# yahoo/bftkv

Hardware: NVIDIA H100
Metric: rsa2048_signature_verifies_per_sec (higher is better)
Workload: dtype u32 limbs / u64 products (integer)

## Files before the change

### bftkv_b200/csrc/rsa_square_r32.cuh

```cuda
#pragma once
#include <cstdint>
#include <cuda_runtime.h>

namespace bftq {
namespace r32 {

__device__ __forceinline__ void mad_pair_first(uint32_t& lo, uint32_t& hi, const uint32_t x, const uint32_t m) {
  asm volatile("mad.lo.cc.u32 %0, %2, %3, %0; madc.hi.cc.u32 %1, %2, %3, %1;" : "+r"(lo), "+r"(hi) : "r"(x), "r"(m));
}
__device__ __forceinline__ void mad_pair_next(uint32_t& lo, uint32_t& hi, const uint32_t x, const uint32_t m) {
  asm volatile("madc.lo.cc.u32 %0, %2, %3, %0; madc.hi.cc.u32 %1, %2, %3, %1;" : "+r"(lo), "+r"(hi) : "r"(x), "r"(m));
}
template <int N>
__device__ __forceinline__ void chain_n(uint32_t* p, uint32_t& c0, uint32_t& c1, const uint32_t* x, const uint32_t m, const uint32_t t) {
  if (N == 0) {
    asm volatile("add.cc.u32 %0, %0, %2; addc.u32 %1, %1, 0;" : "+r"(c0), "+r"(c1) : "r"(t));
    return;
  }
  mad_pair_first(p[0], p[1], x[0], m);
#pragma unroll
  for (int i = 1; i < N; i++) mad_pair_next(p[2 * i], p[2 * i + 1], x[2 * i], m);
  asm volatile("addc.cc.u32 %0, %0, %2; addc.u32 %1, %1, 0;" : "+r"(c0), "+r"(c1) : "r"(t));
}
template <int N>
__device__ __forceinline__ void chain_n1(uint32_t* p, uint32_t& c, const uint32_t* x, const uint32_t m) {
  mad_pair_first(p[0], p[1], x[0], m);
#pragma unroll
  for (int i = 1; i < N; i++) mad_pair_next(p[2 * i], p[2 * i + 1], x[2 * i], m);
  asm volatile("addc.u32 %0, %0, 0;" : "+r"(c));
}

template <int JJ>
__device__ __forceinline__ void sqr_iter(Acc<16>& A, uint32_t& cy1, const uint32_t (&a2)[17], const uint32_t (&n)[16],
                                         const uint32_t n0inv, const int r, const int gbase, const int owner) {
  constexpr int W = 16;
  const uint32_t lt1 = r < owner ? ~1u : 0u, nm = r < owner ? ~0u : ~1u, eqm = r == owner ? ~0u : 0u;
  const uint32_t aj0 = __funnelshift_r(a2[JJ], a2[JJ + 1], 1);
  const uint32_t aj1 = __funnelshift_r(a2[JJ + 1], a2[JJ + 2], 1);
  const uint32_t b0 = __shfl_sync(kFull, aj0, gbase + owner);
  const uint32_t b1 = __shfl_sync(kFull, aj1, gbase + owner);
  uint32_t m0[18], m1[18];
#pragma unroll
  for (int k = 0; k < 17; k++) { m0[k] = a2[k]; m1[k] = a2[k]; }
  m0[17] = 0u; m1[17] = 0u;
  m0[JJ] = (a2[JJ] & lt1) | (aj0 & eqm);
  m0[JJ + 1] = a2[JJ + 1] & nm;
  m1[JJ + 1] = (a2[JJ + 1] & lt1) | (aj1 & eqm);
  uint32_t top1 = a2[16];
  if (JJ + 2 < W) m1[JJ + 2] = a2[JJ + 2] & nm;
  else top1 = a2[16] & (lt1 >> 1);
  const uint32_t t0 = (0u - a2[16]) & b0;
  const uint32_t t1 = (0u - top1) & b1;
  chain_n<(W - JJ) / 2>(A.E + JJ, A.E[W], A.E[W + 1], m0 + JJ, b0, t0);
  uint32_t q0 = A.E[0] * n0inv;
  q0 = __shfl_sync(kFull, q0, gbase);
  chain_n<(W - JJ) / 2>(A.O + JJ, A.O[W], A.O[W + 1], m0 + JJ + 1, b0, 0u);
  chain_n<(W - JJ - 2) / 2>(A.O + JJ + 2, A.O[W], A.O[W + 1], m1 + JJ + 2, b1, t1);
  chain_n1<(W - JJ) / 2>(A.E + JJ + 2, A.O[W + 1], m1 + JJ + 1, b1);
  mac_off0_even_nocin(A, n, q0);
  mac_off0_odd(A, n, q0);
  uint32_t q1 = (A.E[1] + A.O[0] + cy1) * n0inv;
  q1 = __shfl_sync(kFull, q1, gbase);
  Chain<W>::run_cin(A.O, A.O[W], A.O[W + 1], n, q1, cy1);
  chain_n1<W / 2>(A.E + 2, A.O[W + 1], n + 1, q1);
  const uint32_t p0 = A.E[0];
  uint32_t p1, e0;
  asm("add.cc.u32 %0, %3, %4; addc.cc.u32 %1, %5, %6; addc.u32 %2, 0, 0;"
      : "=r"(p1), "=r"(e0), "=r"(cy1) : "r"(A.E[1]), "r"(A.O[0]), "r"(A.E[2]), "r"(A.O[1]));
  uint32_t r0 = __shfl_down_sync(kFull, p0, 1, T);
  uint32_t r1 = __shfl_down_sync(kFull, p1, 1, T);
  if (r == T - 1) { r0 = 0u; r1 = 0u; }
#pragma unroll
  for (int k = 1; k < W; k++) A.E[k] = A.E[k + 2];
  A.E[0] = e0; A.E[W] = 0u; A.E[W + 1] = 0u;
#pragma unroll
  for (int k = 0; k < W; k++) A.O[k] = A.O[k + 2];
  A.O[W] = 0u; A.O[W + 1] = 0u;
  asm volatile("add.cc.u32 %0, %0, %3; addc.cc.u32 %1, %1, %4; addc.u32 %2, %2, 0;"
               : "+r"(A.E[W - 2]), "+r"(A.E[W - 1]), "+r"(A.O[W - 1]) : "r"(r0), "r"(r1));
}

__device__ __forceinline__ void mont_sqr(uint32_t (&out)[16], const uint32_t (&a)[16], const uint32_t (&n)[16], const uint32_t n0inv,
                                         const int r, const int gbase) {
  constexpr int W = 16;
  uint32_t a2[17];
  a2[0] = a[0] << 1;
#pragma unroll
  for (int k = 1; k < W; k++) a2[k] = __funnelshift_l(a[k - 1], a[k], 1);
  a2[16] = a[W - 1] >> 31;
  Acc<W> A;
#pragma unroll
  for (int k = 0; k < W + 4; k++) A.E[k] = 0u;
#pragma unroll
  for (int k = 0; k < W + 2; k++) A.O[k] = 0u;
  uint32_t cy1 = 0u;
#pragma unroll 2
  for (int owner = 0; owner < T; owner++) {
    sqr_iter<0>(A, cy1, a2, n, n0inv, r, gbase, owner);
    sqr_iter<2>(A, cy1, a2, n, n0inv, r, gbase, owner);
    sqr_iter<4>(A, cy1, a2, n, n0inv, r, gbase, owner);
    sqr_iter<6>(A, cy1, a2, n, n0inv, r, gbase, owner);
    sqr_iter<8>(A, cy1, a2, n, n0inv, r, gbase, owner);
    sqr_iter<10>(A, cy1, a2, n, n0inv, r, gbase, owner);
    sqr_iter<12>(A, cy1, a2, n, n0inv, r, gbase, owner);
    sqr_iter<14>(A, cy1, a2, n, n0inv, r, gbase, owner);
  }
  asm volatile("add.cc.u32 %0, %0, %1;" : "+r"(A.O[0]) : "r"(cy1));
#pragma unroll
  for (int k = 1; k < W; k++) asm volatile("addc.cc.u32 %0, %0, 0;" : "+r"(A.O[k]));
  mont_finish(out, A, 0u, 0u, n, r, gbase);
}

}
}
```

### bftkv_b200/csrc/rsa_verify_r32.cuh

```cuda
#pragma once
#include <cstdint>
#include <cuda_runtime.h>
#include "rsa_verify.cuh"

namespace bftq {
namespace r32 {

constexpr int T = 4;

#define BFTQ_CHAIN8_BODY(first)                                                              \
  first " %0, %18, %26, %0;  madc.hi.cc.u32 %1, %18, %26, %1;"                                \
  "madc.lo.cc.u32 %2, %19, %26, %2;  madc.hi.cc.u32 %3, %19, %26, %3;"                        \
  "madc.lo.cc.u32 %4, %20, %26, %4;  madc.hi.cc.u32 %5, %20, %26, %5;"                        \
  "madc.lo.cc.u32 %6, %21, %26, %6;  madc.hi.cc.u32 %7, %21, %26, %7;"                        \
  "madc.lo.cc.u32 %8, %22, %26, %8;  madc.hi.cc.u32 %9, %22, %26, %9;"                        \
  "madc.lo.cc.u32 %10, %23, %26, %10; madc.hi.cc.u32 %11, %23, %26, %11;"                     \
  "madc.lo.cc.u32 %12, %24, %26, %12; madc.hi.cc.u32 %13, %24, %26, %13;"                     \
  "madc.lo.cc.u32 %14, %25, %26, %14; madc.hi.cc.u32 %15, %25, %26, %15;"                     \
  "addc.cc.u32 %16, %16, 0; addc.u32 %17, %17, 0;"
#define BFTQ_CHAIN8_OPS(p, c0, c1, x)                                                                                     \
  : "+r"(p[0]), "+r"(p[1]), "+r"(p[2]), "+r"(p[3]), "+r"(p[4]), "+r"(p[5]), "+r"(p[6]), "+r"(p[7]), "+r"(p[8]), "+r"(p[9]), \
    "+r"(p[10]), "+r"(p[11]), "+r"(p[12]), "+r"(p[13]), "+r"(p[14]), "+r"(p[15]), "+r"(c0), "+r"(c1)                      \
  : "r"(x[0]), "r"(x[2]), "r"(x[4]), "r"(x[6]), "r"(x[8]), "r"(x[10]), "r"(x[12]), "r"(x[14]), "r"(m)

#define BFTQ_CHAIN4_BODY(first)                                                              \
  first " %0, %10, %14, %0;  madc.hi.cc.u32 %1, %10, %14, %1;"                                \
  "madc.lo.cc.u32 %2, %11, %14, %2;  madc.hi.cc.u32 %3, %11, %14, %3;"                        \
  "madc.lo.cc.u32 %4, %12, %14, %4;  madc.hi.cc.u32 %5, %12, %14, %5;"                        \
  "madc.lo.cc.u32 %6, %13, %14, %6;  madc.hi.cc.u32 %7, %13, %14, %7;"                        \
  "addc.cc.u32 %8, %8, 0; addc.u32 %9, %9, 0;"
#define BFTQ_CHAIN4_OPS(p, c0, c1, x)                                                                                     \
  : "+r"(p[0]), "+r"(p[1]), "+r"(p[2]), "+r"(p[3]), "+r"(p[4]), "+r"(p[5]), "+r"(p[6]), "+r"(p[7]), "+r"(c0), "+r"(c1)      \
  : "r"(x[0]), "r"(x[2]), "r"(x[4]), "r"(x[6]), "r"(m)

template <int W>
struct Acc {
  uint32_t E[W + 4];
  uint32_t O[W + 2];
};

template <int W> struct Chain;
template <> struct Chain<16> {
  static __device__ __forceinline__ void run(uint32_t* p, uint32_t& c0, uint32_t& c1, const uint32_t* x, const uint32_t m) {
    asm volatile(BFTQ_CHAIN8_BODY("mad.lo.cc.u32") BFTQ_CHAIN8_OPS(p, c0, c1, x));
  }
  static __device__ __forceinline__ void run_cin(uint32_t* p, uint32_t& c0, uint32_t& c1, const uint32_t* x, const uint32_t m, const uint32_t cin) {
    asm volatile("{ .reg .u32 t; add.cc.u32 t, %27, 0xffffffff;" BFTQ_CHAIN8_BODY("madc.lo.cc.u32") "}"
                 BFTQ_CHAIN8_OPS(p, c0, c1, x), "r"(cin));
  }
};
template <> struct Chain<8> {
  static __device__ __forceinline__ void run(uint32_t* p, uint32_t& c0, uint32_t& c1, const uint32_t* x, const uint32_t m) {
    asm volatile(BFTQ_CHAIN4_BODY("mad.lo.cc.u32") BFTQ_CHAIN4_OPS(p, c0, c1, x));
  }
  static __device__ __forceinline__ void run_cin(uint32_t* p, uint32_t& c0, uint32_t& c1, const uint32_t* x, const uint32_t m, const uint32_t cin) {
    asm volatile("{ .reg .u32 t; add.cc.u32 t, %15, 0xffffffff;" BFTQ_CHAIN4_BODY("madc.lo.cc.u32") "}"
                 BFTQ_CHAIN4_OPS(p, c0, c1, x), "r"(cin));
  }
};

template <int W>
__device__ __forceinline__ void mac_off0_even(Acc<W>& A, const uint32_t (&x)[W], const uint32_t m, const uint32_t cin) {
  Chain<W>::run_cin(A.E, A.E[W], A.E[W + 1], x, m, cin);
}
template <int W>
__device__ __forceinline__ void mac_off0_even_nocin(Acc<W>& A, const uint32_t (&x)[W], const uint32_t m) {
  Chain<W>::run(A.E, A.E[W], A.E[W + 1], x, m);
}
template <int W>
__device__ __forceinline__ void mac_off0_odd(Acc<W>& A, const uint32_t (&x)[W], const uint32_t m) {
  Chain<W>::run(A.O, A.O[W], A.O[W + 1], x + 1, m);
}
template <int W>
__device__ __forceinline__ void mac_off1_even(Acc<W>& A, const uint32_t (&x)[W], const uint32_t m) {
  Chain<W>::run(A.O, A.O[W], A.O[W + 1], x, m);
}
template <int W>
__device__ __forceinline__ void mac_off1_odd(Acc<W>& A, const uint32_t (&x)[W], const uint32_t m) {
  Chain<W>::run(A.E + 2, A.E[W + 2], A.E[W + 3], x + 1, m);
}

template <int W>
__device__ __forceinline__ uint32_t ripple_add(uint32_t (&v)[W], const uint32_t x) {
  uint32_t c;
  asm volatile("add.cc.u32 %0, %0, %1;" : "+r"(v[0]) : "r"(x));
#pragma unroll
  for (int k = 1; k < W; k++) asm volatile("addc.cc.u32 %0, %0, 0;" : "+r"(v[k]));
  asm volatile("addc.u32 %0, 0, 0;" : "=r"(c));
  return c;
}
template <int W>
__device__ __forceinline__ uint32_t ripple_sub(uint32_t (&v)[W], const uint32_t x) {
  uint32_t b;
  asm volatile("sub.cc.u32 %0, %0, %1;" : "+r"(v[0]) : "r"(x));
#pragma unroll
  for (int k = 1; k < W; k++) asm volatile("subc.cc.u32 %0, %0, 0;" : "+r"(v[k]));
  asm volatile("subc.u32 %0, 0, 0;" : "=r"(b));
  return b & 1u;
}
template <int W>
__device__ __forceinline__ uint32_t sub_n(uint32_t (&d)[W], const uint32_t (&v)[W], const uint32_t (&n)[W]) {
  uint32_t b;
  asm volatile("sub.cc.u32 %0, %1, %2;" : "=r"(d[0]) : "r"(v[0]), "r"(n[0]));
#pragma unroll
  for (int k = 1; k < W; k++) asm volatile("subc.cc.u32 %0, %1, %2;" : "=r"(d[k]) : "r"(v[k]), "r"(n[k]));
  asm volatile("subc.u32 %0, 0, 0;" : "=r"(b));
  return b & 1u;
}

__device__ __forceinline__ uint32_t lane_carry_in(const uint32_t gbits, const uint32_t pbits, const int r, uint32_t& out) {
  const uint32_t c1 = gbits & 1u;
  const uint32_t c2 = ((gbits >> 1) & 1u) | (((pbits >> 1) & 1u) & c1);
  const uint32_t c3 = ((gbits >> 2) & 1u) | (((pbits >> 2) & 1u) & c2);
  out = ((gbits >> 3) & 1u) | (((pbits >> 3) & 1u) & c3);
  return r == 0 ? 0u : (r == 1 ? c1 : (r == 2 ? c2 : c3));
}

template <int W, bool CT = false>
__device__ __forceinline__ void mont_finish(uint32_t (&out)[W], Acc<W>& A, const uint32_t cin, const uint32_t Z, const uint32_t (&n)[W],
                                            const int r, const int gbase) {
  uint32_t v[W], hi;
  asm volatile("add.cc.u32 %0, %1, %2;" : "=r"(v[0]) : "r"(A.E[0]), "r"(Z));
#pragma unroll
  for (int k = 1; k < W; k++) asm volatile("addc.cc.u32 %0, %1, %2;" : "=r"(v[k]) : "r"(A.E[k]), "r"(A.O[k - 1]));
  asm volatile("addc.u32 %0, %1, %2;" : "=r"(hi) : "r"(A.E[W]), "r"(A.O[W - 1]));
  uint32_t from_below = __shfl_up_sync(kFull, hi, 1, T);
  if (r == 0) from_below = 0u;
  const uint32_t g = ripple_add(v, from_below + cin);
  bool ones = true;
#pragma unroll
  for (int k = 0; k < W; k++) ones = ones && (v[k] == 0xffffffffu);
  const uint32_t gb = __ballot_sync(kFull, g != 0u) >> gbase;
  const uint32_t pb = __ballot_sync(kFull, ones) >> gbase;
  uint32_t ctop;
  const uint32_t ci = lane_carry_in(gb, pb, r, ctop);
  ripple_add(v, ci);
  const uint32_t top_hi = __shfl_sync(kFull, hi, gbase + T - 1);
  const bool overflow = (top_hi + ctop) != 0u;
  if (CT || __any_sync(kFull, overflow)) {
    uint32_t d[W];
    const uint32_t bo = sub_n(d, v, n);
    bool zeros = true;
#pragma unroll
    for (int k = 0; k < W; k++) zeros = zeros && (d[k] == 0u);
    const uint32_t bgb = __ballot_sync(kFull, bo != 0u) >> gbase;
    const uint32_t bpb = __ballot_sync(kFull, zeros) >> gbase;
    uint32_t btop;
    const uint32_t bi = lane_carry_in(bgb, bpb, r, btop);
    ripple_sub(d, bi);
    if (CT) {
      const uint32_t m = 0u - (uint32_t)overflow;
#pragma unroll
      for (int k = 0; k < W; k++) v[k] = (d[k] & m) | (v[k] & ~m);
    } else if (overflow) {
#pragma unroll
      for (int k = 0; k < W; k++) v[k] = d[k];
    }
  }
#pragma unroll
  for (int k = 0; k < W; k++) out[k] = v[k];
}

template <int W, bool CT = false>
__device__ __forceinline__ void mont_mul(uint32_t (&out)[W], const uint32_t (&a)[W], const uint32_t (&b)[W],
                                         const uint32_t (&n)[W], const uint32_t n0inv, const int r, const int gbase,
                                         const int owners = T) {
  Acc<W> A;
#pragma unroll
  for (int k = 0; k < W + 4; k++) A.E[k] = 0u;
#pragma unroll
  for (int k = 0; k < W + 2; k++) A.O[k] = 0u;
  uint32_t cin = 0u;
  uint32_t Z = 0u;
#pragma unroll 1
  for (int owner = 0; owner < T; owner++) {
    if (owner == owners) break;
    const int src = gbase + owner;
#pragma unroll
    for (int jj = 0; jj < W; jj += 2) {
      const uint32_t b0 = __shfl_sync(kFull, b[jj], src);
      const uint32_t b1 = __shfl_sync(kFull, b[jj + 1], src);
      mac_off0_even(A, a, b0, cin);
      uint32_t q0 = (A.E[0] + Z) * n0inv;
      q0 = __shfl_sync(kFull, q0, gbase);
      mac_off0_odd(A, a, b0);
      mac_off1_even(A, a, b1);
      mac_off1_odd(A, a, b1);
      mac_off0_even_nocin(A, n, q0);
      mac_off0_odd(A, n, q0);
      const uint64_t s0 = (uint64_t)A.E[0] + Z;
      const uint32_t p0 = (uint32_t)s0, c0 = (uint32_t)(s0 >> 32);
      uint32_t q1 = (A.E[1] + A.O[0] + c0) * n0inv;
      q1 = __shfl_sync(kFull, q1, gbase);
      mac_off1_even(A, n, q1);
      mac_off1_odd(A, n, q1);
      const uint64_t s1 = (uint64_t)A.E[1] + A.O[0] + c0;
      const uint32_t p1 = (uint32_t)s1;
      cin = (uint32_t)(s1 >> 32);
      Z = A.O[1];
      uint32_t r0 = __shfl_down_sync(kFull, p0, 1, T);
      uint32_t r1 = __shfl_down_sync(kFull, p1, 1, T);
      if (r == T - 1) { r0 = 0u; r1 = 0u; }
#pragma unroll
      for (int k = 0; k < W + 2; k++) A.E[k] = A.E[k + 2];
      A.E[W + 2] = 0u; A.E[W + 3] = 0u;
#pragma unroll
      for (int k = 0; k < W; k++) A.O[k] = A.O[k + 2];
      A.O[W] = 0u; A.O[W + 1] = 0u;
      asm volatile("add.cc.u32 %0, %0, %4; addc.cc.u32 %1, %1, %5; addc.cc.u32 %2, %2, 0; addc.u32 %3, %3, 0;"
                   : "+r"(A.E[W - 2]), "+r"(A.E[W - 1]), "+r"(A.E[W]), "+r"(A.E[W + 1]) : "r"(r0), "r"(r1));
    }
  }
  mont_finish<W, CT>(out, A, cin, Z, n, r, gbase);
}

template <int W>
__device__ __forceinline__ bool group_ge(const uint32_t (&x)[W], const uint32_t (&n)[W], const int gbase) {
  bool gt = false, lt = false;
#pragma unroll
  for (int j = W - 1; j >= 0; j--) {
    if (!gt && !lt) { gt = x[j] > n[j]; lt = x[j] < n[j]; }
  }
  const uint32_t gmask = ((1u << T) - 1u) << gbase;
  const uint32_t gtb = __ballot_sync(kFull, gt) & gmask;
  const uint32_t ltb = __ballot_sync(kFull, lt) & gmask;
  return gtb >= ltb;
}

template <int W>
__device__ __forceinline__ uint32_t group_sub(uint32_t (&d)[W], const uint32_t (&x)[W], const uint32_t (&y)[W], const int r, const int gbase) {
  const uint32_t bo = sub_n(d, x, y);
  bool zeros = true;
#pragma unroll
  for (int k = 0; k < W; k++) zeros = zeros && (d[k] == 0u);
  const uint32_t bgb = __ballot_sync(kFull, bo != 0u) >> gbase;
  const uint32_t bpb = __ballot_sync(kFull, zeros) >> gbase;
  uint32_t btop;
  const uint32_t bi = lane_carry_in(bgb, bpb, r, btop);
  ripple_sub(d, bi);
  return btop;
}

template <int W>
__device__ __forceinline__ void cond_sub(uint32_t (&x)[W], const uint32_t (&n)[W], const int r, const int gbase) {
  const bool ge = group_ge(x, n, gbase);
  uint32_t d[W];
  group_sub(d, x, n, r, gbase);
  if (ge) {
#pragma unroll
    for (int k = 0; k < W; k++) x[k] = d[k];
  }
}

}
}
#include "rsa_square_r32.cuh"
namespace bftq {
namespace r32 {

struct RsaKey32 {
  uint32_t n[64];
  uint32_t c16[64];
  uint32_t hc16[64];
  uint32_t c32[64];
  uint32_t hc32[64];
  uint32_t n0inv;
  uint32_t e;
  uint32_t nbits;
  uint32_t pad;
};

constexpr int kK1Block = 128, kK1MinBlocks = 4;

__global__ void __launch_bounds__(kK1Block, kK1MinBlocks)
rsa_verify_r32_kernel(const RsaKey32* __restrict__ keys, const uint32_t nkeys, const uint32_t* __restrict__ key_idx,
                      const uint8_t* __restrict__ sig, const uint8_t* __restrict__ digest, const uint32_t hash_alg,
                      const uint64_t n_items, const uint32_t flags, const uint8_t* __restrict__ pre_status,
                      uint8_t* __restrict__ status) {
  constexpr int W = 16;
  constexpr int kGroupsPerWarp = 32 / T;
  __shared__ uint32_t y_s[W][kK1Block];
  __shared__ int nbmax_s;
  const int lane = threadIdx.x & 31;
  const int r = lane & (T - 1);
  const int gbase = lane & ~(T - 1);
  const int plen = c_hash_prefix[hash_alg].len;
  const int dlen = c_hash_prefix[hash_alg].dlen;
  const bool wide = plen + dlen > 63;
  const int check_owners = wide ? 2 : 1;
  const uint64_t warps_total = (uint64_t)gridDim.x * (kK1Block / 32);
  const uint32_t gmask = ((1u << T) - 1u) << gbase;

  for (uint64_t bbase = (uint64_t)blockIdx.x * (kK1Block / 32) * kGroupsPerWarp; bbase < n_items; bbase += warps_total * kGroupsPerWarp) {
    const uint64_t wbase = bbase + (uint64_t)(threadIdx.x >> 5) * kGroupsPerWarp;
    __syncthreads();
    const uint64_t item_raw = wbase + (uint64_t)(lane / T);
    const bool valid = item_raw < n_items;
    const uint64_t item = valid ? item_raw : (n_items - 1);
    uint32_t kidx = __ldg(key_idx + item);
    const bool known = kidx < nkeys;
    if (!known) kidx = 0u;
    const RsaKey32* __restrict__ key = keys + kidx;

    uint32_t nd[W], y[W], t[W];
#pragma unroll
    for (int j = 0; j < W; j++) nd[j] = __ldg(&key->n[r * W + j]);
    const uint32_t n0inv = __ldg(&key->n0inv);
    const uint32_t e = __ldg(&key->e);
    const uint8_t* sp = sig + item * (uint64_t)kRsaBytes;
    const uint8_t* dp = digest + item * (uint64_t)dlen;
    const uint32_t* ck = wide ? key->c32 : key->c16;
    bool s_ge_n;
#pragma unroll
    for (int j = 0; j < W; j++) y[j] = be_word(sp, r * W + j);
    s_ge_n = group_ge(y, nd, gbase);
    const int nb = 32 - __clz(e);
    int nbmax = nb;
#pragma unroll
    for (int o = 16; o >= 1; o >>= 1) nbmax = max(nbmax, __shfl_xor_sync(kFull, nbmax, o));
    if (threadIdx.x == 0) nbmax_s = 0;
    __syncthreads();
    if (lane == 0) atomicMax(&nbmax_s, nbmax);
    __syncthreads();
    nbmax = nbmax_s;
    int bit = nbmax - 2, op = bit >= 0 ? 1 : 3;
#pragma unroll 1
    for (;;) {
      if (op == 1) {
        mont_sqr(t, y, nd, n0inv, r, gbase);
        __syncthreads();
        if (bit <= nb - 2) {
#pragma unroll
          for (int j = 0; j < W; j++) y[j] = t[j];
        }
        const bool mul = bit <= nb - 2 && ((e >> bit) & 1u);
        if (__any_sync(kFull, mul)) op = 2;
        else { bit--; op = bit >= 0 ? 1 : 3; }
      } else {
        uint32_t bop[W];
        if (op == 3) {
#pragma unroll 1
          for (int j = 0; j < W; j++) y_s[j][threadIdx.x] = em_word(r * W + j, dp, plen, dlen, hash_alg);
#pragma unroll
          for (int j = 0; j < W; j++) { bop[j] = y_s[j][threadIdx.x]; y_s[j][threadIdx.x] = y[j]; y[j] = __ldg(&ck[r * W + j]); }
        } else {
#pragma unroll
          for (int j = 0; j < W; j++) bop[j] = be_word(sp, r * W + j);
        }
        mont_mul(t, y, bop, nd, n0inv, r, gbase, op == 2 ? T : check_owners);
        if (op == 3) break;
        if (bit <= nb - 2 && ((e >> bit) & 1u)) {
#pragma unroll
          for (int j = 0; j < W; j++) y[j] = t[j];
        }
        bit--;
        op = bit >= 0 ? 1 : 3;
      }
    }
#pragma unroll
    for (int j = 0; j < W; j++) y[j] = y_s[j][threadIdx.x];
    cond_sub(y, nd, r, gbase);
    cond_sub(t, nd, r, gbase);
    uint32_t d[W];
    const uint32_t b = group_sub(d, y, t, r, gbase);
    const uint32_t* hk = wide ? key->hc32 : key->hc16;
#pragma unroll
    for (int j = 0; j < W; j++) y[j] = __ldg(&hk[r * W + j]);
    group_sub(t, y, d, r, gbase);
    bool eq = true;
#pragma unroll
    for (int j = 0; j < W; j++) eq = eq && (t[j] == (b ? nd[j] : 0u));
    const uint32_t eqb = __ballot_sync(kFull, eq) & gmask;
    if (valid && r == 0) {
      uint8_t st = (eqb == gmask) ? (uint8_t)0 : (uint8_t)1;
      if ((flags & 1u) && s_ge_n) st = 1;
      if (__ldg(&key->nbits) != 2048u) st = 1;
      if (!known) st = 4;
      if (pre_status != nullptr) {
        const uint8_t pre = __ldg(pre_status + item_raw);
        if (pre != 0) st = pre;
      }
      status[item_raw] = st;
    }
  }
}

}
}
```

Before: 59.09 million.

## Square in place, skip idle carry resolution, cache constant padding words

Montgomery squaring now writes straight into its input and, when the result is not committed, rebuilds the original operand from the doubled copy. This removes the separate t-to-y copy. The carry-propagation ballots in mont_finish are skipped when no lane generated a carry. The constant prefix and padding words of the encoded message are computed once per block into shared memory, so only the digest bytes are loaded per item. The neighbour shuffle now uses a precomputed absolute source lane instead of a segmented shuffle_down with a predicate, which relies on the wrapped-in value from the next group being harmless.

```diff
diff --git a/bftkv_b200/csrc/rsa_square_r32.cuh b/bftkv_b200/csrc/rsa_square_r32.cuh
--- a/bftkv_b200/csrc/rsa_square_r32.cuh
+++ b/bftkv_b200/csrc/rsa_square_r32.cuh
@@ -32,7 +32,7 @@
 
 template <int JJ>
 __device__ __forceinline__ void sqr_iter(Acc<16>& A, uint32_t& cy1, const uint32_t (&a2)[17], const uint32_t (&n)[16],
-                                         const uint32_t n0inv, const int r, const int gbase, const int owner) {
+                                         const uint32_t n0inv, const int r, const int gbase, const int up, const int owner) {
   constexpr int W = 16;
   const uint32_t lt1 = r < owner ? ~1u : 0u, nm = r < owner ? ~0u : ~1u, eqm = r == owner ? ~0u : 0u;
   const uint32_t aj0 = __funnelshift_r(a2[JJ], a2[JJ + 1], 1);
@@ -67,9 +67,8 @@
   uint32_t p1, e0;
   asm("add.cc.u32 %0, %3, %4; addc.cc.u32 %1, %5, %6; addc.u32 %2, 0, 0;"
       : "=r"(p1), "=r"(e0), "=r"(cy1) : "r"(A.E[1]), "r"(A.O[0]), "r"(A.E[2]), "r"(A.O[1]));
-  uint32_t r0 = __shfl_down_sync(kFull, p0, 1, T);
-  uint32_t r1 = __shfl_down_sync(kFull, p1, 1, T);
-  if (r == T - 1) { r0 = 0u; r1 = 0u; }
+  const uint32_t r0 = __shfl_sync(kFull, p0, up);
+  const uint32_t r1 = __shfl_sync(kFull, p1, up);
 #pragma unroll
   for (int k = 1; k < W; k++) A.E[k] = A.E[k + 2];
   A.E[0] = e0; A.E[W] = 0u; A.E[W + 1] = 0u;
@@ -80,9 +79,10 @@
                : "+r"(A.E[W - 2]), "+r"(A.E[W - 1]), "+r"(A.O[W - 1]) : "r"(r0), "r"(r1));
 }
 
-__device__ __forceinline__ void mont_sqr(uint32_t (&out)[16], const uint32_t (&a)[16], const uint32_t (&n)[16], const uint32_t n0inv,
-                                         const int r, const int gbase) {
+__device__ __forceinline__ void mont_sqr(uint32_t (&a)[16], const uint32_t (&n)[16], const uint32_t n0inv, const int r, const int gbase,
+                                         const bool commit) {
   constexpr int W = 16;
+  const int up = (gbase + r + 1) & 31;
   uint32_t a2[17];
   a2[0] = a[0] << 1;
 #pragma unroll
@@ -96,19 +96,23 @@
   uint32_t cy1 = 0u;
 #pragma unroll 2
   for (int owner = 0; owner < T; owner++) {
-    sqr_iter<0>(A, cy1, a2, n, n0inv, r, gbase, owner);
-    sqr_iter<2>(A, cy1, a2, n, n0inv, r, gbase, owner);
-    sqr_iter<4>(A, cy1, a2, n, n0inv, r, gbase, owner);
-    sqr_iter<6>(A, cy1, a2, n, n0inv, r, gbase, owner);
-    sqr_iter<8>(A, cy1, a2, n, n0inv, r, gbase, owner);
-    sqr_iter<10>(A, cy1, a2, n, n0inv, r, gbase, owner);
-    sqr_iter<12>(A, cy1, a2, n, n0inv, r, gbase, owner);
-    sqr_iter<14>(A, cy1, a2, n, n0inv, r, gbase, owner);
+    sqr_iter<0>(A, cy1, a2, n, n0inv, r, gbase, up, owner);
+    sqr_iter<2>(A, cy1, a2, n, n0inv, r, gbase, up, owner);
+    sqr_iter<4>(A, cy1, a2, n, n0inv, r, gbase, up, owner);
+    sqr_iter<6>(A, cy1, a2, n, n0inv, r, gbase, up, owner);
+    sqr_iter<8>(A, cy1, a2, n, n0inv, r, gbase, up, owner);
+    sqr_iter<10>(A, cy1, a2, n, n0inv, r, gbase, up, owner);
+    sqr_iter<12>(A, cy1, a2, n, n0inv, r, gbase, up, owner);
+    sqr_iter<14>(A, cy1, a2, n, n0inv, r, gbase, up, owner);
   }
   asm volatile("add.cc.u32 %0, %0, %1;" : "+r"(A.O[0]) : "r"(cy1));
 #pragma unroll
   for (int k = 1; k < W; k++) asm volatile("addc.cc.u32 %0, %0, 0;" : "+r"(A.O[k]));
-  mont_finish(out, A, 0u, 0u, n, r, gbase);
+  mont_finish(a, A, 0u, 0u, n, r, gbase);
+  if (!commit) {
+#pragma unroll
+    for (int k = 0; k < W; k++) a[k] = __funnelshift_r(a2[k], a2[k + 1], 1);
+  }
 }
 
 }
diff --git a/bftkv_b200/csrc/rsa_verify_r32.cuh b/bftkv_b200/csrc/rsa_verify_r32.cuh
--- a/bftkv_b200/csrc/rsa_verify_r32.cuh
+++ b/bftkv_b200/csrc/rsa_verify_r32.cuh
@@ -127,14 +127,16 @@
   uint32_t from_below = __shfl_up_sync(kFull, hi, 1, T);
   if (r == 0) from_below = 0u;
   const uint32_t g = ripple_add(v, from_below + cin);
-  bool ones = true;
-#pragma unroll
-  for (int k = 0; k < W; k++) ones = ones && (v[k] == 0xffffffffu);
-  const uint32_t gb = __ballot_sync(kFull, g != 0u) >> gbase;
-  const uint32_t pb = __ballot_sync(kFull, ones) >> gbase;
-  uint32_t ctop;
-  const uint32_t ci = lane_carry_in(gb, pb, r, ctop);
-  ripple_add(v, ci);
+  uint32_t ctop = 0u;
+  if (CT || __any_sync(kFull, g != 0u)) {
+    bool ones = true;
+#pragma unroll
+    for (int k = 0; k < W; k++) ones = ones && (v[k] == 0xffffffffu);
+    const uint32_t gb = __ballot_sync(kFull, g != 0u) >> gbase;
+    const uint32_t pb = __ballot_sync(kFull, ones) >> gbase;
+    const uint32_t ci = lane_carry_in(gb, pb, r, ctop);
+    ripple_add(v, ci);
+  }
   const uint32_t top_hi = __shfl_sync(kFull, hi, gbase + T - 1);
   const bool overflow = (top_hi + ctop) != 0u;
   if (CT || __any_sync(kFull, overflow)) {
@@ -280,6 +282,7 @@
   constexpr int W = 16;
   constexpr int kGroupsPerWarp = 32 / T;
   __shared__ uint32_t y_s[W][kK1Block];
+  __shared__ uint32_t em_s[2 * W];
   __shared__ int nbmax_s;
   const int lane = threadIdx.x & 31;
   const int r = lane & (T - 1);
@@ -290,6 +293,7 @@
   const int check_owners = wide ? 2 : 1;
   const uint64_t warps_total = (uint64_t)gridDim.x * (kK1Block / 32);
   const uint32_t gmask = ((1u << T) - 1u) << gbase;
+  if (threadIdx.x < 2 * W) em_s[threadIdx.x] = 4 * (int)threadIdx.x >= dlen ? em_word((int)threadIdx.x, digest, plen, dlen, hash_alg) : 0u;
 
   for (uint64_t bbase = (uint64_t)blockIdx.x * (kK1Block / 32) * kGroupsPerWarp; bbase < n_items; bbase += warps_total * kGroupsPerWarp) {
     const uint64_t wbase = bbase + (uint64_t)(threadIdx.x >> 5) * kGroupsPerWarp;
@@ -327,22 +331,25 @@
 #pragma unroll 1
     for (;;) {
       if (op == 1) {
-        mont_sqr(t, y, nd, n0inv, r, gbase);
+        mont_sqr(y, nd, n0inv, r, gbase, bit <= nb - 2);
         __syncthreads();
-        if (bit <= nb - 2) {
-#pragma unroll
-          for (int j = 0; j < W; j++) y[j] = t[j];
-        }
         const bool mul = bit <= nb - 2 && ((e >> bit) & 1u);
         if (__any_sync(kFull, mul)) op = 2;
         else { bit--; op = bit >= 0 ? 1 : 3; }
       } else {
         uint32_t bop[W];
         if (op == 3) {
-#pragma unroll 1
-          for (int j = 0; j < W; j++) y_s[j][threadIdx.x] = em_word(r * W + j, dp, plen, dlen, hash_alg);
-#pragma unroll
-          for (int j = 0; j < W; j++) { bop[j] = y_s[j][threadIdx.x]; y_s[j][threadIdx.x] = y[j]; y[j] = __ldg(&ck[r * W + j]); }
+#pragma unroll
+          for (int j = 0; j < W; j++) {
+            const int w = r * W + j;
+            bop[j] = em_s[w & (2 * W - 1)];
+            if (4 * w < dlen) {
+              const uint8_t* p = dp + (dlen - 4 - 4 * w);
+              bop[j] = __byte_perm(__byte_perm(__ldg(p + 3), __ldg(p + 2), 0x3340), __byte_perm(__ldg(p + 1), __ldg(p), 0x3340), 0x5410);
+            }
+            y_s[j][threadIdx.x] = y[j];
+            y[j] = __ldg(&ck[r * W + j]);
+          }
         } else {
 #pragma unroll
           for (int j = 0; j < W; j++) bop[j] = be_word(sp, r * W + j);
```

Measured after the change: 59.98 million (median of 6 runs). 1.5% higher.
